# fomalhautb/KM-BART

Hardware: AMD Instinct MI355X
Metric: train_tokens_per_sec (higher is better)
Workload: dtype bf16

## Files before the change

km-bart_amd/csrc/gemm.hip:

```cpp
#include <algorithm>
#include <cstdio>
#include <cstdlib>
#include <cstring>
#include <map>
#include <tuple>
#include <vector>
#include <type_traits>
#include "common.h"
#include "diag.h"
#include "kernels.h"

#ifdef KMB_GEMM_STAMP
#ifndef KMB_STAMP_SLOTS
#define KMB_STAMP_SLOTS 8
#endif
__device__ unsigned long long* g_kmb_stamps = nullptr;
extern "C" int kmb_debug_set_stamps(void* p) {
  return (int)hipMemcpyToSymbol(HIP_SYMBOL(g_kmb_stamps), &p, sizeof(p));
}
#define KMB_STAMP(i)                                                                                   \
  do {                                                                                                 \
    if (g_kmb_stamps != nullptr && threadIdx.x == 0)                                                   \
      g_kmb_stamps[(size_t)blockIdx.x * KMB_STAMP_SLOTS + (i)] = __builtin_amdgcn_s_memrealtime();                   \
  } while (0)
// ... 1033 lines not shown
      __builtin_amdgcn_sched_group_barrier(0x100, NDA, 3);
      __builtin_amdgcn_sched_group_barrier(0x008, 2, 3);
#pragma unroll
      for (int q = 0; q < 2; ++q) {
        __builtin_amdgcn_sched_group_barrier(0x010, 2, 3);
        __builtin_amdgcn_sched_group_barrier(0x008, 6, 3);
      }
    }
    __builtin_amdgcn_sched_barrier(0);
  };
  using Yes = std::true_type;
  using No = std::false_type;
  int t = 0;
  for (; t + 2 < nt; ++t) kstep(t, Yes{}, Yes{});
  if (t + 1 < nt) { kstep(t, No{}, Yes{}); ++t; }
  kstep(t, No{}, No{});
  __syncthreads();
  KMB_STAMP(2);
  KMB_STAMP_VALUE(5, kmb_wait_ticks);
  if (KMB_DIAG_BIT(p.tile_order, 512)) {
    float keep = 0.f;
#pragma unroll
    for (int i = 0; i < 8; ++i)
#pragma unroll
      for (int j = 0; j < 4; ++j) keep += acc[i][j][0];
    if (keep == 1.2345e30f) p.out_bf16[0] = 0;
    return;
  }
  float* ef = reinterpret_cast<float*>(smem);
  for (int h = 0; h < 2; ++h) {
    if ((wn >> 1) == h) {
#pragma unroll
      for (int i = 0; i < 8; ++i)
#pragma unroll
        for (int j = 0; j < 4; ++j)
#pragma unroll
          for (int q = 0; q < 4; ++q)
            ef[(wm * 128 + i * 16 + g * 4 + q) * EPI_LD + (wn & 1) * 64 + j * 16 + r] = acc[i][j][q];
    }
    __syncthreads();
    if (h == 0) KMB_STAMP(3);
    gemm_epilogue_phase2<512, false>(p, ef, reinterpret_cast<float*>(smem + 2 * EPI_BYTES), tid, row0, col0 + h * 128, slice);
    __syncthreads();
  }
  KMB_STAMP(4);
}


#ifndef KMB_GEMM_DEVICE_ONLY
constexpr int VR = 320, VN = 256;
constexpr int VK = 32;
constexpr int V_A = VR * VK * 2;
constexpr int V_STG = (VR + VN) * VK * 2;
constexpr int V_NSTG = 4;
constexpr int LDS_VOC = V_NSTG * V_STG;

template <bool STATS>
__global__ __launch_bounds__(512) void gemm_kernel_allrows(const KmbGemm p, float* __restrict__ stats) {
  extern __shared__ __attribute__((aligned(16))) char smem[];
  const int tid = threadIdx.x;
  const int lane = tid & 63, wave = __builtin_amdgcn_readfirstlane(tid >> 6);
  const int wm = wave >> 2, wn = wave & 3;
  const int r = lane & 15, g = lane >> 4;
  const int col0 = (int)blockIdx.x * VN;
  f32x4 acc[10][4];
#pragma unroll
  for (int i = 0; i < 10; ++i)
#pragma unroll
    for (int j = 0; j < 4; ++j) acc[i][j] = f32x4{0.f, 0.f, 0.f, 0.f};
  const int ns = p.K / VK;
  const int prow = lane >> 2, pchunk = (lane & 3) ^ ((0 - (lane >> 4)) & 3);
  uint32_t offA[3], offB[2];
#pragma unroll
  for (int i = 0; i < 3; ++i) {
    const int row = (wave + 8 * i) * 16 + prow;
    const int grow = row < p.M ? row : p.M - 1;
    offA[i] = (uint32_t)((grow * p.lda + pchunk * 8) * 2);
  }
#pragma unroll
  for (int i = 0; i < 2; ++i) {
    const int col = col0 + (2 * wave + i) * 16 + prow;
    const int gcol = col < p.N ? col : p.N - 1;
    offB[i] = (uint32_t)(((gcol - col0) * p.ldb + pchunk * 8) * 2);
  }
  auto uniform_ptr = [](const char* ptr) {
    const uint64_t a = reinterpret_cast<uint64_t>(ptr);
    const uint32_t lo = __builtin_amdgcn_readfirstlane((uint32_t)a);
    const uint32_t hi = __builtin_amdgcn_readfirstlane((uint32_t)(a >> 32));
    return reinterpret_cast<const char*>(((uint64_t)hi << 32) | lo);
  };
  const char* const gA = reinterpret_cast<const char*>(p.A);
  const char* const gB = reinterpret_cast<const char*>(p.B) + (size_t)col0 * p.ldb * 2;
  auto dma_stage = [&](int s) {
    char* st = smem + (s & (V_NSTG - 1)) * V_STG;
    const char* ga = uniform_ptr(gA + (size_t)s * VK * 2);
    const char* gb = uniform_ptr(gB + (size_t)s * VK * 2);
    dma_piece(ga, offA[0], st + wave * 1024);
    dma_piece(ga, offA[1], st + (wave + 8) * 1024);
    if (wave < 4) dma_piece(ga, offA[2], st + (wave + 16) * 1024);
    dma_piece(gb, offB[0], st + V_A + (2 * wave) * 1024);
    dma_piece(gb, offB[1], st + V_A + (2 * wave + 1) * 1024);
  };
  KMB_STAMP(0);
  KMB_STAMP_ID();
#ifdef KMB_GEMM_STAMP
  const uint64_t kmb_c0 = __builtin_amdgcn_s_memtime(), kmb_r0 = __builtin_amdgcn_s_memrealtime();
#endif
  dma_stage(0);
  if (ns > 1) dma_stage(1);
  if (ns > 2) dma_stage(2);
  const int frag_off = r * 64 + ((g ^ ((0 - (r >> 2)) & 3)) << 4);
  for (int s = 0; s < ns; ++s) {
    const int newer = ns - 1 - s;
    if (wave < 4) {
      if (newer >= 2) __builtin_amdgcn_s_waitcnt(0x0F7A);
      else if (newer == 1) __builtin_amdgcn_s_waitcnt(0x0F75);
      else __builtin_amdgcn_s_waitcnt(0x0F70);
    } else {
      if (newer >= 2) __builtin_amdgcn_s_waitcnt(0x0F78);
      else if (newer == 1) __builtin_amdgcn_s_waitcnt(0x0F74);
      else __builtin_amdgcn_s_waitcnt(0x0F70);
    }
    __builtin_amdgcn_s_barrier();
    if (s == 0) KMB_STAMP(1);
    if (s == ns / 2) KMB_STAMP(3);
    const bool more = s + 3 < ns;
    char* nst = smem + ((s + 3) & (V_NSTG - 1)) * V_STG;
    const char* ga = uniform_ptr(gA + (size_t)(s + 3) * VK * 2);
    const char* gb = uniform_ptr(gB + (size_t)(s + 3) * VK * 2);
    const char* cur = smem + (s & (V_NSTG - 1)) * V_STG + frag_off;
    bf16x8 fb[4], fa[10];
#pragma unroll
    for (int j = 0; j < 4; ++j) fb[j] = *reinterpret_cast<const bf16x8*>(cur + V_A + (wn * 4 + j) * 1024);
#pragma unroll
    for (int i = 0; i < 10; ++i) fa[i] = *reinterpret_cast<const bf16x8*>(cur + (wm * 10 + i) * 1024);
#pragma unroll
    for (int i = 0; i < 10; ++i) {
#pragma unroll
      for (int j = 0; j < 4; ++j) acc[i][j] = __builtin_amdgcn_mfma_f32_16x16x32_bf16(fb[j], fa[i], acc[i][j], 0, 0, 0);
      if (more && (i & 1)) {
        if (i == 1) dma_piece(gb, offB[0], nst + V_A + (2 * wave) * 1024);
        if (i == 3) dma_piece(ga, offA[0], nst + wave * 1024);
        if (i == 5) dma_piece(gb, offB[1], nst + V_A + (2 * wave + 1) * 1024);
        if (i == 7) dma_piece(ga, offA[1], nst + (wave + 8) * 1024);
        if (i == 9 && wave < 4) dma_piece(ga, offA[2], nst + (wave + 16) * 1024);
      }
    }
  }
  __syncthreads();
  KMB_STAMP(2);
#ifdef KMB_GEMM_STAMP
  KMB_STAMP_VALUE(5, __builtin_amdgcn_s_memtime() - kmb_c0);
  KMB_STAMP_VALUE(6, __builtin_amdgcn_s_memrealtime() - kmb_r0);
#endif
  if constexpr (!STATS) {
#pragma unroll
    for (int j = 0; j < 4; ++j) {
      const int col = col0 + wn * 64 + j * 16 + g * 4;
      if (col >= p.N) continue;
      f32x4 b4 = {0.f, 0.f, 0.f, 0.f};
      if (p.bias != nullptr) b4 = *reinterpret_cast<const f32x4*>(p.bias + col);
#pragma unroll
      for (int i = 0; i < 10; ++i) {
        const int row = wm * 160 + i * 16 + r;
        if (row < p.M) *reinterpret_cast<f32x4*>(p.out_f32 + (size_t)row * p.ld_out_f32 + col) = acc[i][j] + b4;
      }
    }
  } else {
    float* smax = reinterpret_cast<float*>(smem);
    float* ssum = smax + VR * 4;
    f32x4 b4[4];
    bool inside[4];
#pragma unroll
    for (int j = 0; j < 4; ++j) {
      const int col = col0 + wn * 64 + j * 16 + g * 4;
      inside[j] = col < p.N;
      b4[j] = f32x4{0.f, 0.f, 0.f, 0.f};
      if (p.bias != nullptr && inside[j]) b4[j] = *reinterpret_cast<const f32x4*>(p.bias + col);
    }
    const bool ragged = col0 + VN > p.N;
#pragma unroll
    for (int i = 0; i < 10; ++i) {
      float lm = -INFINITY;
#pragma unroll
      for (int j = 0; j < 4; ++j) {
        acc[i][j] = acc[i][j] + b4[j];
        if (ragged && !inside[j]) acc[i][j] = f32x4{-INFINITY, -INFINITY, -INFINITY, -INFINITY};
        lm = fmaxf(fmaxf(lm, fmaxf(acc[i][j][0], acc[i][j][1])), fmaxf(acc[i][j][2], acc[i][j][3]));
      }
      lm = fmaxf(lm, __shfl_xor(lm, 16, 64));
      lm = fmaxf(lm, __shfl_xor(lm, 32, 64));
      if (g == 0) smax[(wm * 160 + i * 16 + r) * 4 + wn] = lm;
    }
    __syncthreads();
#pragma unroll
    for (int i = 0; i < 10; ++i) {
      const int row = wm * 160 + i * 16 + r;
      const f32x4 m4 = *reinterpret_cast<const f32x4*>(smax + row * 4);
      const float m = fmaxf(fmaxf(m4[0], m4[1]), fmaxf(m4[2], m4[3]));
      float sum = 0.f;
#pragma unroll
      for (int j = 0; j < 4; ++j) {
        if (row < p.M && inside[j])
          *reinterpret_cast<f32x4*>(p.out_f32 + (size_t)row * p.ld_out_f32 + col0 + wn * 64 + j * 16 + g * 4) = acc[i][j];
#pragma unroll
        for (int q = 0; q < 4; ++q) sum += __expf(acc[i][j][q] - m);
      }
      sum += __shfl_xor(sum, 16, 64);
      sum += __shfl_xor(sum, 32, 64);
      if (g == 0) ssum[row * 4 + wn] = sum;
    }
    __syncthreads();
    if (tid < p.M) {
      const f32x4 m4 = *reinterpret_cast<const f32x4*>(smax + tid * 4);
      const f32x4 s4 = *reinterpret_cast<const f32x4*>(ssum + tid * 4);
      float2 ms;
      ms.x = fmaxf(fmaxf(m4[0], m4[1]), fmaxf(m4[2], m4[3]));
      ms.y = (s4[0] + s4[1]) + (s4[2] + s4[3]);
      reinterpret_cast<float2*>(stats)[(size_t)tid * gridDim.x + blockIdx.x] = ms;
    }
  }
  KMB_STAMP(4);
}

#endif

template <bool KC, int NP = 8>
__device__ __forceinline__ void dma_offsets256w4(uint32_t (&off)[NP], int ld, int r0, int R, int wave, int lane) {
#pragma unroll
  for (int i = 0; i < NP; ++i) {
    const int piece = wave * NP + i;
    if (KC) {
      const int row = piece * 8 + (lane >> 3);
      const int c = (lane & 7) ^ ((row >> 1) & 7);
      int grow = r0 + row;
      grow = grow < R ? grow : R - 1;
      off[i] = (uint32_t)(((grow - r0) * ld + c * 8) * 2);
    } else {
      const int krow = piece * 2 + (lane >> 5);
      const int ps = lane & 31;
      const int c32 = (ps >> 1) ^ swz_nkc(krow);
      int m = r0 + c32 * 16 + (ps & 1) * 8;
      const int mlast = ((R - 1) >> 3) << 3;
      m = m < R ? m : mlast;
      off[i] = (uint32_t)((krow * ld + (m - r0)) * 2);
    }
  }
}

constexpr int EPW_BYTES = 16 * 128 * 4;
constexpr int LDS11 = 2 * ST4 + 4 * EPW_BYTES;
constexpr int LDS12 = 2 * (BM4 + 128) * BK * 2 + 4 * EPW_BYTES;

template <int ACT, bool RES, bool CS, bool FAST, int WROWS, int NJ = 8>
__device__ __forceinline__ void v11_epilogue(const KmbGemm& p, f32x4 (&acc)[8][NJ], float* ef, int lane, int r, int g,
                                             int row0w, int col0w) {
  constexpr int WCOLS = NJ * 16;
  constexpr int LDE = WCOLS > 64 ? 128 : 64;
  float csum[8];
#pragma unroll
  for (int e = 0; e < 8; ++e) csum[e] = 0.f;
  float* const wbase = ef + r * LDE;
  const int sw = (r & 7) << 3;
  auto stage = [&](const f32x4 (&a)[NJ]) {
#pragma unroll
    for (int j = 0; j < NJ; ++j) *reinterpret_cast<f32x4*>(wbase + ((j * 16 + g * 4) ^ sw)) = a[j];
    asm volatile("" ::: "memory");
  };
#pragma unroll 1
  for (int i = 0; i < WROWS / 16; ++i) {
    switch (i) {
      case 0: stage(acc[0]); break;
      case 1: stage(acc[1]); break;
      case 2: stage(acc[2]); break;
      case 3: stage(acc[3]); break;
      case 4: stage(acc[4]); break;
      case 5: stage(acc[5]); break;
      case 6: stage(acc[6]); break;
      default: stage(acc[7]); break;
    }
    gemm_epilogue_body<64, (WCOLS > 64), 4, LDE, true, 128, ACT, RES, CS, FAST, true, WCOLS>(p, ef, nullptr, lane, row0w + i * 16,
                                                                                    col0w, csum);
  }
  if (CS && (ACT >= 0 || p.colsum != nullptr)) {
#pragma unroll
    for (int e = 0; e < 8; ++e) {
      csum[e] += __shfl_xor(csum[e], 16);
      csum[e] += __shfl_xor(csum[e], 32);
    }
    if (lane < WCOLS / 8) {
      const int prow = row0w >> 6;
      const int c8 = lane * 8;
#pragma unroll
      for (int e = 0; e < 8; ++e) {
        if (FAST || col0w + c8 + e < p.N) {
          p.colsum[(size_t)prow * p.N + col0w + c8 + e] = csum[e];
          if (WROWS == 128 && (FAST || row0w + 64 < p.M)) p.colsum[(size_t)(prow + 1) * p.N + col0w + c8 + e] = 0.f;
        }
      }
    }
  }
}

template <bool BIAS, bool SCALE, int ACT, bool RES, bool DROP, bool CS, int WROWS, bool F32 = false, int NJ = 8>
__device__ __forceinline__ void v11_epilogue_lean(const KmbGemm& p, f32x4 (&acc)[8][NJ], float* ef, int lane, int r, int g,
                                                  int row0w, int col0w) {
  constexpr int WCOLS = NJ * 16;
  constexpr int CL = WCOLS > 64 ? 16 : 8, RPI = 64 / CL, NIT = 16 / RPI, LDE = WCOLS > 64 ? 128 : 64;
  const int lr = lane / CL;
  const int c8 = ((lane % CL) * 8 < WCOLS) ? (lane % CL) * 8 : WCOLS - 8;
  const int gcol = col0w + c8;
  kmb_f32x2 bias2[4], csum2[4];
#pragma unroll
  for (int e = 0; e < 4; ++e) {
    bias2[e] = BIAS ? kmb_f32x2{p.bias[gcol + 2 * e], p.bias[gcol + 2 * e + 1]} : kmb_f32x2{0.f, 0.f};
    csum2[e] = kmb_f32x2{0.f, 0.f};
  }
  const kmb_f32x2 scale2 = {p.col_scale, p.col_scale};
  const kmb_f32x2 dscale2 = {p.drop_scale, p.drop_scale};
  float* const wbase = ef + r * LDE;
  const int sw = (r & 7) << 2;
  auto stage = [&](const f32x4 (&a)[NJ]) {
#pragma unroll
    for (int j = 0; j < NJ; ++j) *reinterpret_cast<f32x4*>(wbase + ((j * 16 + g * 4) ^ sw)) = a[j];
    asm volatile("" ::: "memory");
  };
  const float* rd[NIT];
#pragma unroll
  for (int it = 0; it < NIT; ++it)
    rd[it] = ef + (lr + RPI * it) * LDE + (c8 ^ (((lr + RPI * it) & 7) << 2));
  const int rd_hi = (lr & 1) ? -4 : 4;
  bf16_t* out = F32 ? nullptr : p.out_bf16 + (size_t)(row0w + lr) * p.ld_out_bf16 + gcol;
  float* out32 = F32 ? p.out_f32 + (size_t)(row0w + lr) * p.ld_out_f32 + gcol : nullptr;
  bf16_t* pre = (ACT == 1 && p.preact != nullptr) ? p.preact + (size_t)(row0w + lr) * p.ld_preact + gcol : nullptr;
  const bf16_t* side = nullptr;
  size_t ld_side = 0;
  if (RES) { side = p.residual + (size_t)(row0w + lr) * p.ld_res + gcol; ld_side = (size_t)p.ld_res; }
  if (ACT == 2) { side = p.aux + (size_t)(row0w + lr) * p.ld_aux + gcol; ld_side = (size_t)p.ld_aux; }
  constexpr bool SIDE = RES || ACT == 2;
  static_assert(!(RES && ACT == 2), "one side stream");
  constexpr bool PAIRS = NIT == 4;
  constexpr int AHEAD = PAIRS ? 2 : 1;
  u32x4 sE[NIT];
  [[maybe_unused]] u32x4 sO[NIT];
  if (SIDE) {
#pragma unroll
    for (int it = 0; it < NIT; ++it) {
      sE[it] = *reinterpret_cast<const u32x4*>(side + (size_t)(RPI * it) * ld_side);
      if constexpr (PAIRS) sO[it] = *reinterpret_cast<const u32x4*>(side + (size_t)(16 + RPI * it) * ld_side);
    }
  }
  float hE[NIT];
  [[maybe_unused]] float hO[NIT];
  const float* shift_base = ACT == 5 ? p.row_shift + row0w + lr : nullptr;
  if constexpr (ACT == 5) {
#pragma unroll
    for (int it = 0; it < NIT; ++it) {
      hE[it] = shift_base[RPI * it];
      if constexpr (PAIRS) hO[it] = shift_base[16 + RPI * it];
    }
  }
  auto stage_chunk = [&](int i) {
    switch (i) {
      case 0: stage(acc[0]); break;
      case 1: stage(acc[1]); break;
      case 2: stage(acc[2]); break;
      case 3: stage(acc[3]); break;
      case 4: stage(acc[4]); break;
      case 5: stage(acc[5]); break;
      case 6: stage(acc[6]); break;
      default: stage(acc[7]); break;
    }
  };
  static_assert((WROWS / 16) % 2 == 0, "chunks are walked in pairs");
  auto chunk = [&](const int i, u32x4 (&sv)[NIT], float (&hv)[NIT]) {
    [[maybe_unused]] float su[SIDE ? NIT : 1][8];
    [[maybe_unused]] float hc[ACT == 5 ? NIT : 1];
    const int ahead = i + AHEAD < WROWS / 16 ? i + AHEAD : WROWS / 16 - 1;
    if (SIDE) {
#pragma unroll
      for (int it = 0; it < NIT; ++it) unpack8(sv[it], su[it]);
      __builtin_amdgcn_sched_barrier(0);
#pragma unroll
      for (int it = 0; it < NIT; ++it) sv[it] = *reinterpret_cast<const u32x4*>(side + (size_t)(16 * ahead + RPI * it) * ld_side);
    }
    if constexpr (ACT == 5) {
#pragma unroll
      for (int it = 0; it < NIT; ++it) hc[it] = hv[it];
#pragma unroll
      for (int it = 0; it < NIT; ++it) asm volatile("" : "+v"(hc[it]));
      __builtin_amdgcn_sched_barrier(0);
#pragma unroll
      for (int it = 0; it < NIT; ++it) hv[it] = shift_base[16 * ahead + RPI * it];
    }
    f32x4 lo4[NIT], hi4[NIT];
#pragma unroll
    for (int it = 0; it < NIT; ++it) {
      lo4[it] = *reinterpret_cast<const f32x4*>(rd[it]);
      hi4[it] = *reinterpret_cast<const f32x4*>(rd[it] + rd_hi);
    }
    asm volatile("" ::: "memory");
    if (i + 1 < WROWS / 16) stage_chunk(i + 1);
#pragma unroll
    for (int it = 0; it < NIT; ++it) {
      const f32x4 lo = lo4[it];
      const f32x4 hi = hi4[it];
      kmb_f32x2 v[4] = {{lo[0], lo[1]}, {lo[2], lo[3]}, {hi[0], hi[1]}, {hi[2], hi[3]}};
#pragma unroll
      for (int e = 0; e < 4; ++e) {
        if (BIAS) v[e] = v[e] + bias2[e];
        if (SCALE) v[e] = v[e] * scale2;
      }
      const size_t roff = (size_t)(16 * i + RPI * it);
      if constexpr (ACT == 5) {
        static_assert(ACT != 5 || WCOLS == 64 || WCOLS == 128, "act 5: 64- or 128-column wave blocks");
        const int grow = row0w + lr + 16 * i + RPI * it;
        const float c = hc[it];
        const kmb_f32x2 c2 = {c, c};
#pragma unroll
        for (int e = 0; e < 4; ++e) v[e] = v[e] - c2;
        if (p.pick_col != nullptr) {
          const int rel = (int)((long long)p.pick_col[grow] - (long long)gcol);
          if (rel >= 0 && rel < 8) {
            float picked = 0.f;
#pragma unroll
            for (int e = 0; e < 4; ++e) {
              if (rel == 2 * e) picked = v[e][0];
              if (rel == 2 * e + 1) picked = v[e][1];
            }
            p.pick_out[grow] = picked;
          }
        }
#pragma unroll
        for (int e = 0; e < 4; ++e) {
          const kmb_f32x2 t = v[e] * 1.4426950408889634f;
          v[e] = kmb_f32x2{__builtin_amdgcn_exp2f(fminf(t[0], 115.f)), __builtin_amdgcn_exp2f(fminf(t[1], 115.f))};
        }
        float sum = (v[0][0] + v[0][1]) + (v[1][0] + v[1][1]) + ((v[2][0] + v[2][1]) + (v[3][0] + v[3][1]));
#pragma unroll
        for (int o = 1; o < CL; o <<= 1) sum += __shfl_xor(sum, o);
        if ((lane % CL) == 0) {
          float* slot = p.row_sums + (size_t)grow * p.row_sums_ld + (col0w >> 6);
          slot[0] = sum;
          if (WCOLS == 128) slot[1] = 0.f;
        }
      } else if (ACT == 1) {
        if (pre != nullptr) {
          kmb_f32x2 dv[4];
#pragma unroll
          for (int e = 0; e < 4; ++e) {
            kmb_f32x2 y;
            gelu_both2(v[e], y, dv[e]);
            v[e] = y;
          }
          const u32x4 pk = {pack2bf(dv[0][0], dv[0][1]), pack2bf(dv[1][0], dv[1][1]), pack2bf(dv[2][0], dv[2][1]), pack2bf(dv[3][0], dv[3][1])};
          KMB_NT_STORE(pk, reinterpret_cast<u32x4*>(pre + roff * p.ld_preact));
        } else {
#pragma unroll
          for (int e = 0; e < 4; ++e) v[e] = gelu2(v[e]);
        }
      } else if (ACT == 2) {
#pragma unroll
        for (int e = 0; e < 4; ++e) v[e] = v[e] * kmb_f32x2{su[it][2 * e], su[it][2 * e + 1]};
      }
      if (DROP) {
        const uint32_t grow = (uint32_t)(row0w + lr + 16 * i + RPI * it);
#pragma unroll
        for (int e = 0; e < 4; ++e) {
          const kmb_f32x2 kept = v[e] * dscale2;
          v[e][0] = drop_keep(p.drop_seed, grow, (uint32_t)(gcol + 2 * e), p.drop_thr16) ? kept[0] : 0.f;
          v[e][1] = drop_keep(p.drop_seed, grow, (uint32_t)(gcol + 2 * e + 1), p.drop_thr16) ? kept[1] : 0.f;
        }
      }
      if (RES) {
#pragma unroll
        for (int e = 0; e < 4; ++e) v[e] = v[e] + kmb_f32x2{su[it][2 * e], su[it][2 * e + 1]};
      }
      if (CS) {
#pragma unroll
        for (int e = 0; e < 4; ++e) csum2[e] = csum2[e] + v[e];
      }
      if (F32) {
        float* o = out32 + roff * p.ld_out_f32;
        KMB_NT_STORE((f32x4{v[0][0], v[0][1], v[1][0], v[1][1]}), reinterpret_cast<f32x4*>(o));
        KMB_NT_STORE((f32x4{v[2][0], v[2][1], v[3][0], v[3][1]}), reinterpret_cast<f32x4*>(o + 4));
      } else {
        const u32x4 pk = {pack2bf(v[0][0], v[0][1]), pack2bf(v[1][0], v[1][1]), pack2bf(v[2][0], v[2][1]), pack2bf(v[3][0], v[3][1])};
#ifdef KMB_PLAIN_FFN_OUT
        if (ACT == 1 || ACT == 2) *reinterpret_cast<u32x4*>(out + roff * p.ld_out_bf16) = pk;
        else KMB_NT_STORE(pk, reinterpret_cast<u32x4*>(out + roff * p.ld_out_bf16));
#else
        KMB_NT_STORE(pk, reinterpret_cast<u32x4*>(out + roff * p.ld_out_bf16));
#endif
      }
    }
  };
  stage_chunk(0);
  if constexpr (PAIRS) {
#pragma unroll 1
    for (int i = 0; i < WROWS / 16; i += 2) {
      chunk(i, sE, hE);
      chunk(i + 1, sO, hO);
    }
  } else {
#pragma unroll 1
    for (int i = 0; i < WROWS / 16; ++i) chunk(i, sE, hE);
  }
  if (CS) {
    float csum[8];
#pragma unroll
    for (int e = 0; e < 4; ++e) { csum[2 * e] = csum2[e][0]; csum[2 * e + 1] = csum2[e][1]; }
#pragma unroll
    for (int e = 0; e < 8; ++e) {
      if (CL == 8) csum[e] += __shfl_xor(csum[e], 8);
      csum[e] += __shfl_xor(csum[e], 16);
      csum[e] += __shfl_xor(csum[e], 32);
    }
    if (lane < CL) {
      const int prow = row0w >> 6;
#pragma unroll
      for (int e = 0; e < 8; ++e) {
        p.colsum[(size_t)prow * p.N + gcol + e] = csum[e];
        if (WROWS == 128) p.colsum[(size_t)(prow + 1) * p.N + gcol + e] = 0.f;
      }
    }
  }
}

template <bool A_KC, bool B_KC, int BNT, int NW = 4>
__global__ __launch_bounds__(NW * 64) __attribute__((amdgpu_waves_per_eu(NW / 4, NW / 4)))
void gemm_kernel_v11(const KmbGemm p, uint32_t* sched, int dyn_first) {
  static_assert(NW == 4 || (NW == 8 && (BNT == 256 || BNT == 192)), "eight waves: 256 x 256 and 256 x 192 tiles only");
  extern __shared__ __attribute__((aligned(16))) char smem[];
  KMB_STAMP(0);
  KMB_STAMP_ID();
  [[maybe_unused]] uint64_t kmb_loop_ticks = 0, kmb_epi_ticks = 0, kmb_wait_ticks = 0, kmb_drain_ticks = 0;
  const int tid = threadIdx.x;
  const int lane = tid & 63, wave = __builtin_amdgcn_readfirstlane(tid >> 6);
  constexpr int WN = NW == 8 ? 4 : BNT == 128 ? 1 : 2, WM = NW / WN, WROWS = BM4 / WM, MH = WROWS / 64;
  constexpr int WCOLS = BNT / WN, NJ = WCOLS / 16;
  constexpr int BIMG = (BNT == 192 && !B_KC) ? 256 : BNT;
  constexpr int NPA = 32 / NW;
  constexpr int NPB = BIMG / 32 * 4 / NW;
  constexpr int STG = (BM4 + BIMG) * BK * 2;
  const int wm = wave / WN, wn = wave % WN;
  const int r = lane & 15, g = lane >> 4;
  const int tiles_n = (p.N + BNT - 1) / BNT;
  const int tiles_m = (p.M + BM4 - 1) / BM4;
  const int ntiles = tiles_m * tiles_n;
  constexpr int CB = 8;
  const bool col_blocks = (p.tile_order & 8) != 0 && tiles_n > CB;
  const int cb_full = tiles_n / CB;
  auto decode_tile = [&](int t, int& tm, int& tn) {
    if (!col_blocks) { tm = t / tiles_n; tn = t - tm * tiles_n; return; }
    const int blk = t / (CB * tiles_m);
    if (blk < cb_full) {
      const int rem = t - blk * (CB * tiles_m);
      tm = rem / CB; tn = blk * CB + (rem - tm * CB);
    } else {
      const int wl = tiles_n - cb_full * CB;
      const int rem = t - cb_full * (CB * tiles_m);
      tm = rem / wl; tn = cb_full * CB + (rem - tm * wl);
    }
  };
  const int pf_sharers = col_blocks ? CB : tiles_n;
  const bool xcd_ranges = (p.tile_order & 1) != 0;
  const int per = xcd_ranges ? (int)gridDim.x >> 3 : (int)gridDim.x;
  const int xcd = (int)blockIdx.x & 7, loc = (int)blockIdx.x >> 3;
  const int tq = ntiles >> 3, trem = ntiles & 7;
  const int range0 = !xcd_ranges ? 0 : xcd < trem ? xcd * (tq + 1) : trem * (tq + 1) + (xcd - trem) * tq;
  const int range1 = !xcd_ranges ? ntiles : range0 + tq + (xcd < trem ? 1 : 0);
  const int first = xcd_ranges ? range0 + loc : (int)blockIdx.x;
  const bool dyn = sched != nullptr;
  uint32_t* const my_ctr = sched + (xcd_ranges ? xcd : 0);
  auto retire = [&]() {
    if (dyn && tid == 0) {
      if (atomicAdd(sched + 8, 1u) == gridDim.x - 1u) {
#pragma unroll
        for (int i = 0; i < 9; ++i) sched[i] = 0u;
      }
    }
  };
  int* const next_slot = reinterpret_cast<int*>(smem + 2 * STG);
  constexpr int PFW = NW - 1;
  const unsigned touch_lds = kmb_lds_addr(smem + 2 * STG + PFW * (WCOLS > 64 ? EPW_BYTES : EPW_BYTES / 2) + 2048);
  uint32_t fetched = 0u;
  const int dyn_base = (dyn && dyn_first) ? range0 : range0 + per;
  int first_tile = first;
  if (dyn && dyn_first) {
    if (tid == 0) *next_slot = range0 + (int)atomicAdd(my_ctr, 1u);
    __syncthreads();
    first_tile = __builtin_amdgcn_readfirstlane(*next_slot);
    __syncthreads();
  }
  if (first_tile >= range1) { retire(); return; }
#if defined(KMB_GEMM_STAMP) && KMB_STAMP_SLOTS >= 12
  const uint64_t kmb_c0 = __builtin_amdgcn_s_memtime(), kmb_r0 = __builtin_amdgcn_s_memrealtime();
#endif
#ifdef KMB_DIAG
  if (const int stg = (p.tile_order >> 16) & 255) {
    const int q = ((int)blockIdx.x >> 3) & 3;
    for (int i = 0; i < q * stg; ++i) __builtin_amdgcn_s_sleep(18);
  }
#endif
  const int nt = p.K / BK;
  constexpr int A_BYTES = BM4 * BK * 2;
  const size_t stepA = A_KC ? (size_t)BK * 2 : (size_t)BK * p.lda * 2;
  const size_t stepB = B_KC ? (size_t)BK * 2 : (size_t)BK * p.ldb * 2;
  auto uniform_ptr = [](const char* ptr) {
    const uint64_t a = reinterpret_cast<uint64_t>(ptr);
    const uint32_t lo = __builtin_amdgcn_readfirstlane((uint32_t)a);
    const uint32_t hi = __builtin_amdgcn_readfirstlane((uint32_t)(a >> 32));
    return reinterpret_cast<const char*>(((uint64_t)hi << 32) | lo);
  };

  uint32_t offA[NPA], offB[NPB];
  const char *gA_d, *gB_d;
  int tile_d = first_tile, td = 0;
#ifndef KMB_V11_PREFETCH
#define KMB_V11_PREFETCH 1
#endif
#ifndef KMB_V11_PFD
#define KMB_V11_PFD 2
#endif
  constexpr int KMB_PFD = KMB_V11_PFD;
  constexpr bool PF_ON = KMB_V11_PREFETCH != 0 && A_KC;
  const bool pf_rt = (p.tile_order & 2) != 0;
  uint32_t pf_off = 0u, pfn_off = 0u;
  const char* pfn_base = reinterpret_cast<const char*>(p.A);
  bool pf_pending = false, pfn_ok = false;
  auto pf_row_offset = [&](int tn, int row0) {
    int share = (BM4 + pf_sharers - 1) / pf_sharers;
    share = share > 64 ? 64 : share;
    int prow = tn * share + (lane < share ? lane : 0);
    prow = prow < BM4 ? prow : BM4 - 1;
    prow = row0 + prow < p.M ? prow : 0;
    return (uint32_t)prow * (uint32_t)p.lda * 2u;
  };
  auto set_dma_tile = [&](int tile) {
    int tm, tn;
    decode_tile(tile, tm, tn);
    const int row0 = tm * BM4, col0 = tn * BNT;
    if (PF_ON) {
      pf_off = pf_row_offset(col_blocks ? tn % CB : tn, row0);
      const int tx = tile + per;
      pfn_ok = tx < range1;
      if (pfn_ok) {
        int tmx, tnx;
        decode_tile(tx, tmx, tnx);
        pfn_off = pf_row_offset(col_blocks ? tnx % CB : tnx, tmx * BM4);
        pfn_base = uniform_ptr(reinterpret_cast<const char*>(p.A) + (size_t)tmx * BM4 * p.lda * 2);
      }
    }
    dma_offsets256w4<A_KC, NPA>(offA, p.lda, row0, p.M, wave, lane);
    if constexpr (BNT == 128) dma_offsets<B_KC>(offB, p.ldb, col0, p.N, wave, lane);
    else dma_offsets256w4<B_KC, NPB>(offB, p.ldb, col0, p.N, wave, lane);
    gA_d = uniform_ptr(reinterpret_cast<const char*>(p.A) + (A_KC ? (size_t)row0 * p.lda * 2 : (size_t)row0 * 2));
    gB_d = uniform_ptr(reinterpret_cast<const char*>(p.B) + (B_KC ? (size_t)col0 * p.ldb * 2 : (size_t)col0 * 2));
  };
  int tile_next = first_tile;
  auto advance_cursor = [&]() {
    if (td == nt) {
      td = 0;
      tile_next = dyn ? __builtin_amdgcn_readfirstlane(*next_slot) : tile_d + per;
      if (tile_next < range1) tile_d = tile_next;
      set_dma_tile(tile_d);
    }
  };
  char* const dstA = smem + wave * (NPA * 1024);
  char* const dstB = smem + A_BYTES + wave * (NPB * 1024);
#ifndef KMB_V11_SPLIT
#define KMB_V11_SPLIT 1
#endif
  constexpr int NA3 = KMB_V11_SPLIT == 3 ? NPA / 2 : NPA;
  constexpr int NB3 = KMB_V11_SPLIT == 0 ? NPB : 0;
  constexpr int NB0 = KMB_V11_SPLIT == 0 ? 0 : KMB_V11_SPLIT == 2 ? NPB / 2 : NPB;
  constexpr int NB1 = NPB - NB3 - NB0;
  constexpr int P3 = (NA3 + NB3) / 2, P0 = (NPA - NA3 + NB0) / 2, P1 = NB1 / 2;
  auto dma_a = [&](int buf, int lo, int hi) {
    char* da = dstA + buf * STG;
#ifndef KMB_V11_NODMA
#pragma unroll
    for (int i = 0; i < NPA; ++i) {
#ifdef KMB_A_NT
      if (i >= lo && i < hi) { if constexpr (A_KC) dma_piece_nt(gA_d, offA[i], da + i * 1024); else dma_piece(gA_d, offA[i], da + i * 1024); }
#else
      if (i >= lo && i < hi) dma_piece(gA_d, offA[i], da + i * 1024);
#endif
    }
#endif
    if (hi == NPA && lo < hi) gA_d = uniform_ptr(gA_d + stepA);
  };
  auto dma_b = [&](int buf, int lo, int hi) {
    char* db = dstB + buf * STG;
#ifndef KMB_V11_NODMA
#pragma unroll
    for (int i = 0; i < NPB; ++i)
      if (i >= lo && i < hi) dma_piece(gB_d, offB[i], db + i * 1024);
#endif
    if (hi == NPB && lo < hi) {
      gB_d = uniform_ptr(gB_d + stepB);
      ++td;
    }
  };
  auto dma_stage_a = [&](int buf) { dma_a(buf, 0, NPA); };
  auto dma_stage_b = [&](int buf, int) { dma_b(buf, 0, NPB); };

  constexpr int NDA = A_KC ? 4 : 8;
  constexpr int NDB = B_KC ? NJ : 2 * NJ;
  constexpr int NM = 4 * NJ;
  bf16x8 fa[2][4], fb[2][NJ];
  f32x4 acc[8][NJ];
  constexpr bool REMAT = NW == 8;
  const int rm_ka = r * 128 + ((g ^ ((r >> 1) & 7)) << 4);
  const int rm_sw = ((r >> 2) & 3) | ((g & 1) << 2);
  const int rm_l = (g * 8 + (r >> 2)) * (BIMG * 2) + ((r & 3) << 3);
  const int rm_nb = rm_l | (rm_sw << 5);
  const int rm_na = ((g * 8 + (r >> 2)) * (BM4 * 2) + ((r & 3) << 3)) | (rm_sw << 5);
#ifndef KMB_TR_BUILTIN
  constexpr bool TRASM = (BNT == 256 || KMB_TR_ALL) && !(A_KC && B_KC);
#else
  constexpr bool TRASM = false;
#endif
  auto tr_read = [&](const char* ptr) {
#ifndef KMB_TR_BUILTIN
    if constexpr (TRASM) return kmb_tr_read_asm(ptr);
    else
#endif
    return __builtin_amdgcn_ds_read_tr16_b64_v4i16((__attribute__((address_space(3))) s16x4*)ptr);
  };
  auto read_a = [&](const char* stage, int kk, int half, bf16x8 (&dst)[4]) {
    if constexpr (REMAT && A_KC) {
      int c = rm_ka;
      asm volatile("" : "+v"(c));
      const char* base = stage + (c ^ (kk << 6)) + (wm * (MH * 4) + half * 4) * 2048;
#pragma unroll
      for (int i = 0; i < 4; ++i) dst[i] = *reinterpret_cast<const bf16x8*>(base + i * 2048);
    } else if constexpr (REMAT) {
      int c = rm_na;
      asm volatile("" : "+v"(c));
#pragma unroll
      for (int i = 0; i < 4; ++i) {
        const char* pj = stage + kk * (32 * BM4 * 2) + (c ^ ((wm * (MH * 4) + half * 4 + i) << 5));
#pragma unroll
        for (int hh = 0; hh < 2; ++hh) {
          const s16x4 t = tr_read(pj + hh * (4 * BM4 * 2));
          dst[i][hh * 4 + 0] = t[0]; dst[i][hh * 4 + 1] = t[1]; dst[i][hh * 4 + 2] = t[2]; dst[i][hh * 4 + 3] = t[3];
        }
      }
    } else {
#pragma unroll
      for (int i = 0; i < 4; ++i) dst[i] = read_frag3<A_KC, BM4, TRASM>(stage, wm * (MH * 4) + half * 4 + i, kk, r, g);
    }
  };
  auto read_b = [&](const char* stage, int kk, bf16x8 (&dst)[NJ]) {
    if constexpr (REMAT && B_KC) {
      int c = rm_ka;
      asm volatile("" : "+v"(c));
      const char* base = stage + A_BYTES + (c ^ (kk << 6)) + (wn * NJ) * 2048;
#pragma unroll
      for (int j = 0; j < NJ; ++j) dst[j] = *reinterpret_cast<const bf16x8*>(base + j * 2048);
    } else if constexpr (REMAT) {
      int c = rm_nb;
      asm volatile("" : "+v"(c));
#pragma unroll
      for (int j = 0; j < NJ; ++j) {
        const char* pj = stage + A_BYTES + kk * (32 * BIMG * 2) + (c ^ ((wn * NJ + j) << 5));
#pragma unroll
        for (int hh = 0; hh < 2; ++hh) {
          const s16x4 t = tr_read(pj + hh * (4 * BIMG * 2));
          dst[j][hh * 4 + 0] = t[0]; dst[j][hh * 4 + 1] = t[1]; dst[j][hh * 4 + 2] = t[2]; dst[j][hh * 4 + 3] = t[3];
        }
      }
    } else {
#pragma unroll
      for (int j = 0; j < NJ; ++j) dst[j] = read_frag3<B_KC, BIMG, TRASM>(stage + A_BYTES, wn * NJ + j, kk, r, g);
    }
  };
#ifdef KMB_V11_MFMA32_TIMING
  f32x16 acc32[4][4];
  static_assert(NJ == 8, "timing experiment: 128-column wave blocks only");
  auto mma = [&](int half, const bf16x8 (&a)[4], const bf16x8 (&b)[8]) {
#pragma unroll
    for (int ii = 0; ii < 2; ++ii)
#pragma unroll
      for (int jj = 0; jj < 4; ++jj)
#pragma unroll
        for (int ks = 0; ks < 2; ++ks)
          acc32[half * 2 + ii][jj] = __builtin_amdgcn_mfma_f32_32x32x16_bf16(b[jj * 2 + ks], a[ii * 2 + ks], acc32[half * 2 + ii][jj], 0, 0, 0);
  };
#define KMB_MF(n) ((n) / 2)
#else
  auto mma = [&](int half, const bf16x8 (&a)[4], const bf16x8 (&b)[NJ]) {
#pragma unroll
    for (int i = 0; i < 4; ++i)
#pragma unroll
      for (int j = 0; j < NJ; ++j)
        acc[half * 4 + i][j] = __builtin_amdgcn_mfma_f32_16x16x32_bf16(b[j], a[i], acc[half * 4 + i][j], 0, 0, 0);
  };
#define KMB_MF(n) (n)
#endif

  set_dma_tile(tile_d);
  if (PF_ON && pf_rt && wave == PFW) {
#pragma unroll
    for (int i = 2; i < 2 + KMB_PFD; ++i) {
      if (i < nt) {
        const char* pbase = uniform_ptr(gA_d + (size_t)i * stepA);
        KMB_L2_TOUCH(pf_off, pbase, touch_lds);
// ... 915 lines not shown
```

km-bart_amd/csrc/gemm_lean.hip:

```cpp
#define KMB_GEMM_DEVICE_ONLY
#include "gemm.hip"

namespace {

constexpr int LN_STG = (256 + 256) * BK * 2;
constexpr int LN_A = 256 * BK * 2;
constexpr int LN_EPW = 16 * 64 * 4;
constexpr int LN_LDS = 2 * LN_STG + 8 * LN_EPW;

enum { LN_BIAS = 0, LN_BIAS_RES = 1, LN_PLAIN = 2, LN_GELU = 3, LN_DGELU_CS = 4, LN_CE = 5 };

__device__ __forceinline__ const char* ln_uniform(const char* ptr) {
  const uint64_t a = reinterpret_cast<uint64_t>(ptr);
  const uint32_t lo = (uint32_t)__builtin_amdgcn_readfirstlane((uint32_t)a);
  const uint32_t hi = (uint32_t)__builtin_amdgcn_readfirstlane((uint32_t)(a >> 32));
  return reinterpret_cast<const char*>(((uint64_t)hi << 32) | lo);
}

template <bool B_KC, int EC>
__global__ __launch_bounds__(512) __attribute__((amdgpu_waves_per_eu(2, 2))) void gemm_kernel_lean(const KmbGemm p, uint32_t* sched, int dyn_first) {
  extern __shared__ __attribute__((aligned(16))) char smem[];
  const int tid = threadIdx.x;
  const int lane = tid & 63, wave = __builtin_amdgcn_readfirstlane(tid >> 6);
  const int wm = wave >> 2, wn = wave & 3;
  const int r = lane & 15, g = lane >> 4;
  constexpr int NJ = 4;
  const int tiles_n = p.N / 256, tiles_m = p.M / 256;
  const int ntiles = tiles_m * tiles_n;
  constexpr int CB = 8;
  const bool col_blocks = (p.tile_order & 8) != 0 && tiles_n > CB;
  const int cb_full = tiles_n / CB;
  auto decode_tile = [&](int t, int& tm, int& tn) {
    if (!col_blocks) { tm = t / tiles_n; tn = t - tm * tiles_n; return; }
    const int blk = t / (CB * tiles_m);
    if (blk < cb_full) {
      const int rem = t - blk * (CB * tiles_m);
      tm = rem / CB; tn = blk * CB + (rem - tm * CB);
    } else {
      const int wl = tiles_n - cb_full * CB;
      const int rem = t - cb_full * (CB * tiles_m);
      tm = rem / wl; tn = cb_full * CB + (rem - tm * wl);
    }
  };
  const int per = (int)gridDim.x >> 3;
  const int xcd = (int)blockIdx.x & 7, loc = (int)blockIdx.x >> 3;
  const int tq = ntiles >> 3, trem = ntiles & 7;
  const int range0 = xcd < trem ? xcd * (tq + 1) : trem * (tq + 1) + (xcd - trem) * tq;
  const int range1 = range0 + tq + (xcd < trem ? 1 : 0);
  const int nt = p.K / BK;
  const bool dyn = sched != nullptr;
  uint32_t* const my_ctr = sched + xcd;
  auto retire = [&]() {
    if (dyn && tid == 0) {
      if (atomicAdd(sched + 8, 1u) == gridDim.x - 1u) {
#pragma unroll
        for (int i = 0; i < 9; ++i) sched[i] = 0u;
      }
    }
  };
  int* const next_slot = reinterpret_cast<int*>(smem + 2 * LN_STG);
  const int dyn_base = (dyn && dyn_first) ? range0 : range0 + per;
  int first_tile = range0 + loc;
  if (dyn && dyn_first) {
    if (tid == 0) *next_slot = range0 + (int)atomicAdd(my_ctr, 1u);
    __syncthreads();
    first_tile = __builtin_amdgcn_readfirstlane(*next_slot);
    __syncthreads();
  }
  if (first_tile >= range1) { retire(); return; }

  constexpr int NPW = 4;
  constexpr bool TRASM = KMB_TR_ALL && !B_KC;
  uint32_t offA[NPW], offB[NPW];
  dma_offsets256w4<true, 4>(offA, p.lda, 0, 1 << 30, wave, lane);
  dma_offsets256w4<B_KC, 4>(offB, p.ldb, 0, 1 << 30, wave, lane);
  const size_t stepB = B_KC ? (size_t)BK * 2 : (size_t)BK * p.ldb * 2;
  const char *gA_d, *gB_d;
  int tile_d = first_tile, td = 0;
  int tile_next = first_tile;
  constexpr int LN_PFD = 2;
#ifdef KMB_LN_NOTOUCH
  constexpr int TCH = 0;
#else
  constexpr int TCH = 1;
#endif
  const int sharers = col_blocks ? CB : tiles_n;
  const int pf_share = (256 + sharers - 1) / sharers;
  const int pf_gs = (pf_share + 7) >> 3;
  const char *gA_tile, *gA_nx;
  int pf_rows = 0, pf_rows_nx = 0;
  auto set_dma_tile = [&](int tile) {
    int tm, tn;
    decode_tile(tile, tm, tn);
    gA_d = ln_uniform(reinterpret_cast<const char*>(p.A) + (size_t)tm * 256 * p.lda * 2);
    gB_d = ln_uniform(reinterpret_cast<const char*>(p.B) + (B_KC ? (size_t)tn * 256 * p.ldb * 2 : (size_t)tn * 256 * 2));
    gA_tile = gA_d;
    pf_rows = (col_blocks ? tn % CB : tn) * pf_share;
    const int tx = (!dyn && tile + per < range1) ? tile + per : tile;
    decode_tile(tx, tm, tn);
    gA_nx = ln_uniform(reinterpret_cast<const char*>(p.A) + (size_t)tm * 256 * p.lda * 2);
    pf_rows_nx = (col_blocks ? tn % CB : tn) * pf_share;
  };
  const unsigned touch_lds = kmb_lds_addr(smem + 2 * LN_STG + wave * LN_EPW + 2048);
  auto touch = [&](int ahead) {
    const int ps = td + ahead;
    const bool nx = ps >= nt;
    const char* sbase = ln_uniform((nx ? gA_nx : gA_tile) + (size_t)(nx ? ps - nt : ps) * (BK * 2));
    int row = wave * pf_gs + (lane < pf_gs ? lane : pf_gs - 1);
    row = row < pf_share ? row : pf_share - 1;
    row += nx ? pf_rows_nx : pf_rows;
    row = row < 256 ? row : 255;
    const uint32_t voff = (uint32_t)row * (uint32_t)p.lda * 2u;
    KMB_L2_TOUCH(voff, sbase, touch_lds);
  };
  auto dma_stage = [&](char* stage) {
    char* da = stage + wave * 4096;
    char* db = stage + LN_A + wave * 4096;
#pragma unroll
    for (int i = 0; i < 4; ++i) dma_piece(gA_d, offA[i], da + i * 1024);
#pragma unroll
    for (int i = 0; i < 4; ++i) dma_piece(gB_d, offB[i], db + i * 1024);
    gA_d = ln_uniform(gA_d + BK * 2);
    gB_d = ln_uniform(gB_d + stepB);
  };
  auto advance_cursor = [&]() {
    if (++td == nt) {
      td = 0;
      tile_next = dyn ? __builtin_amdgcn_readfirstlane(*next_slot) : tile_d + per;
      if (tile_next < range1) tile_d = tile_next;
      set_dma_tile(tile_d);
    }
  };

  bf16x8 fa[2][4], fb[2][NJ];
  f32x4 acc[8][NJ];
  auto read_a = [&](const char* st, int kk, int half, bf16x8 (&d)[4]) {
#pragma unroll
    for (int i = 0; i < 4; ++i) d[i] = read_frag3<true, 256>(st, wm * 8 + half * 4 + i, kk, r, g);
  };
  [[maybe_unused]] uint32_t bbase[NJ];
  if constexpr (TRASM) {
    const int krow0 = g * 8 + (r >> 2);
#pragma unroll
    for (int j = 0; j < NJ; ++j) bbase[j] = (uint32_t)(LN_A + krow0 * 512 + (((wn * NJ + j) ^ swz_nkc(krow0)) << 5) + ((r & 3) << 3));
  }
  auto read_b = [&](const char* st, auto kk_c, bf16x8 (&d)[NJ]) {
    constexpr int kk = decltype(kk_c)::value;
    if constexpr (TRASM) {
#ifndef KMB_TR_BUILTIN
      const uint32_t sb = (uint32_t)(uintptr_t)(__attribute__((address_space(3))) const char*)st;
#pragma unroll
      for (int j = 0; j < NJ; ++j) {
        const uint32_t a = sb + bbase[j];
        const s16x4 t0 = kmb_tr_read_asm_off<kk * 32 * 512>(a);
        const s16x4 t1 = kmb_tr_read_asm_off<(kk * 32 + 4) * 512>(a);
        d[j][0] = t0[0]; d[j][1] = t0[1]; d[j][2] = t0[2]; d[j][3] = t0[3];
        d[j][4] = t1[0]; d[j][5] = t1[1]; d[j][6] = t1[2]; d[j][7] = t1[3];
      }
#endif
    } else {
#pragma unroll
      for (int j = 0; j < NJ; ++j) d[j] = read_frag3<B_KC, 256, false>(st + LN_A, wn * NJ + j, kk, r, g);
    }
  };
  using K0 = std::integral_constant<int, 0>;
  using K1 = std::integral_constant<int, 1>;
  auto mma = [&](int half, const bf16x8 (&a)[4], const bf16x8 (&b)[NJ]) {
#pragma unroll
    for (int i = 0; i < 4; ++i)
#pragma unroll
      for (int j = 0; j < NJ; ++j)
        acc[half * 4 + i][j] = __builtin_amdgcn_mfma_f32_16x16x32_bf16(b[j], a[i], acc[half * 4 + i][j], 0, 0, 0);
  };
  constexpr int NDA = 4, NDB = B_KC ? NJ : 2 * NJ;
  auto kstep = [&](char* cur, const char* nxt, auto last_c, int w, int ntouch) {
    constexpr bool LAST = decltype(last_c)::value;
    if constexpr (TRASM) KMB_TR_SYNC();
    read_a(cur, 0, 1, fa[1]);
    mma(0, fa[0], fb[0]);
#pragma unroll
    for (int q = 0; q < NDA; ++q) { __builtin_amdgcn_sched_group_barrier(0x008, 2, 0); __builtin_amdgcn_sched_group_barrier(0x100, 1, 0); __builtin_amdgcn_sched_group_barrier(0x008, 2, 0); }
    __builtin_amdgcn_sched_barrier(0);
    if constexpr (TRASM) KMB_TR_SYNC();
    read_b(cur, K1{}, fb[1]);
    read_a(cur, 1, 0, fa[0]);
    mma(1, fa[1], fb[0]);
#pragma unroll
    for (int q = 0; q < 8; ++q) { __builtin_amdgcn_sched_group_barrier(0x008, 2, 1); __builtin_amdgcn_sched_group_barrier(0x100, (NDB + NDA + 7) / 8, 1); }
    __builtin_amdgcn_sched_barrier(0);
    if constexpr (TRASM) KMB_TR_SYNC();
    read_a(cur, 1, 1, fa[1]);
    mma(0, fa[0], fb[1]);
#pragma unroll
    for (int q = 0; q < NDA; ++q) { __builtin_amdgcn_sched_group_barrier(0x008, 2, 2); __builtin_amdgcn_sched_group_barrier(0x100, 1, 2); __builtin_amdgcn_sched_group_barrier(0x008, 2, 2); }
    __builtin_amdgcn_sched_barrier(0);
    if (LAST || w == 0) __builtin_amdgcn_s_waitcnt(0x0070);
    else if (w == 1) __builtin_amdgcn_s_waitcnt(0x0071);
    else __builtin_amdgcn_s_waitcnt(0x0072);
    __builtin_amdgcn_s_barrier();
    __builtin_amdgcn_s_waitcnt(0xC07F);
    __builtin_amdgcn_sched_barrier(0);
    if constexpr (!LAST) {
      read_b(nxt, K0{}, fb[0]);
      read_a(nxt, 0, 0, fa[0]);
    }
    dma_stage(cur);
    mma(1, fa[1], fb[1]);
    if constexpr (!LAST) {
#pragma unroll
      for (int q = 0; q < 8; ++q) { __builtin_amdgcn_sched_group_barrier(0x008, 2, 3); __builtin_amdgcn_sched_group_barrier(0x100, (NDB + NDA + 7) / 8, 3); }
    }
    __builtin_amdgcn_sched_barrier(0);
    if constexpr (!LAST && TCH != 0) {
      if (ntouch >= 1) touch(LN_PFD);
      if (ntouch >= 2) touch(LN_PFD + 2);
      __builtin_amdgcn_sched_barrier(0);
    }
    advance_cursor();
  };
  using Yes = std::true_type;
  using No = std::false_type;
  set_dma_tile(tile_d);
  dma_stage(smem);
  if constexpr (TCH != 0) touch(LN_PFD);
  advance_cursor();
  dma_stage(smem + LN_STG);
  if constexpr (TCH != 0) touch(LN_PFD);
  advance_cursor();
  __builtin_amdgcn_s_waitcnt(TCH ? 0x0F7A : 0x0F78);
  __builtin_amdgcn_s_barrier();
  read_b(smem, K0{}, fb[0]);
  read_a(smem, 0, 0, fa[0]);

  float* const ef = reinterpret_cast<float*>(smem + 2 * LN_STG + wave * LN_EPW);
  int it = 0;
  uint32_t fetched = 0u;
  for (int tile = first_tile; tile < range1; tile = tile_next) {
#pragma unroll
    for (int i = 0; i < 8; ++i)
#pragma unroll
      for (int j = 0; j < NJ; ++j) acc[i][j] = f32x4{0.f, 0.f, 0.f, 0.f};
    int w = 0;
    for (int t = 0; t + 1 < nt; ++t, ++it) {
      if (dyn && t == 1 && tid == 0) fetched = atomicAdd(my_ctr, 1u);
      if (dyn && t == 3 && tid == 0) *next_slot = dyn_base + (int)fetched;
      const int ntouch = TCH == 0 ? 0 : t + 4 < nt ? 1 : t + 2 < nt ? 2 : 0;
      kstep(smem + (it & 1) * LN_STG, smem + ((it + 1) & 1) * LN_STG, No{}, w, ntouch);
      w = ntouch;
    }
    kstep(smem + (it & 1) * LN_STG, smem + ((it + 1) & 1) * LN_STG, Yes{}, 0, 0);
    ++it;
    if constexpr (TRASM) KMB_TR_SYNC();
    if (KMB_DIAG_BIT(p.tile_order, 512)) {
#pragma unroll
      for (int i = 0; i < 8; ++i)
#pragma unroll
        for (int j = 0; j < NJ; ++j) asm volatile("" ::"v"(acc[i][j]));
    } else {
      int tm, tn;
      decode_tile(tile, tm, tn);
      const int row0w = tm * 256 + wm * 128, col0w = tn * 256 + wn * 64;
      const bool hs = col0w < p.col_scale_n, hd = p.drop_thr16 != 0u, hr = p.residual != nullptr;
#define KMB_LN_LEAN(B, S, A, R, D, C) v11_epilogue_lean<B, S, A, R, D, C, 128, false, NJ>(p, acc, ef, lane, r, g, row0w, col0w)
      if constexpr (EC == LN_BIAS) { if (hs) KMB_LN_LEAN(true, true, 0, false, false, false); else KMB_LN_LEAN(true, false, 0, false, false, false); }
      if constexpr (EC == LN_BIAS_RES) { if (hd) KMB_LN_LEAN(true, false, 0, true, true, false); else KMB_LN_LEAN(true, false, 0, true, false, false); }
      if constexpr (EC == LN_PLAIN) { if (hr) KMB_LN_LEAN(false, false, 0, true, false, false); else KMB_LN_LEAN(false, false, 0, false, false, false); }
      if constexpr (EC == LN_GELU) KMB_LN_LEAN(true, false, 1, false, false, false);
      if constexpr (EC == LN_DGELU_CS) KMB_LN_LEAN(false, false, 2, false, false, true);
      if constexpr (EC == LN_CE) KMB_LN_LEAN(true, false, 5, false, false, false);
#undef KMB_LN_LEAN
    }
    __builtin_amdgcn_sched_barrier(0);
    read_b(smem + (it & 1) * LN_STG, K0{}, fb[0]);
    read_a(smem + (it & 1) * LN_STG, 0, 0, fa[0]);
  }
  if constexpr (TRASM) KMB_TR_SYNC();
  __builtin_amdgcn_s_waitcnt(0x0F70);
  retire();
}

int ln_class(const KmbGemm& p) {
  const bool hb = p.bias != nullptr, hr = p.residual != nullptr, hd = p.drop_thr16 != 0u, hc = p.colsum != nullptr;
  const bool hs = p.col_scale_n > 0;
  if (p.act == 0 && hb && !hr && !hd && !hc) return LN_BIAS;
  if (p.act == 0 && hb && hr && !hc && !hs) return LN_BIAS_RES;
  if (p.act == 0 && !hb && !hd && !hc && !hs) return LN_PLAIN;
  if (p.act == 1 && hb && !hr && !hd && !hc && !hs) return LN_GELU;
  if (p.act == 2 && !hb && !hr && !hd && hc && !hs) return LN_DGELU_CS;
  if (p.act == 5 && hb && !hr && !hd && !hc && !hs) return LN_CE;
  return -1;
}

template <bool B_KC>
hipError_t ln_launch_layout(int ec, const KmbGemm& p, dim3 grid, hipStream_t stream, uint32_t* sched, int dyn_first) {
#define KMB_LN_CASE(E)                                                                                                          \
  case E: {                                                                                                                     \
    static bool attr = false;                                                                                                   \
    if (!attr) {                                                                                                                \
      hipError_t e = hipFuncSetAttribute((const void*)gemm_kernel_lean<B_KC, E>, hipFuncAttributeMaxDynamicSharedMemorySize, LN_LDS); \
      if (e != hipSuccess) return e;                                                                                            \
      attr = true;                                                                                                              \
    }                                                                                                                           \
    hipLaunchKernelGGL((gemm_kernel_lean<B_KC, E>), grid, dim3(512), LN_LDS, stream, p, sched, dyn_first);                                         \
    break;                                                                                                                      \
  }
  switch (ec) {
    KMB_LN_CASE(LN_BIAS)
    KMB_LN_CASE(LN_BIAS_RES)
    KMB_LN_CASE(LN_PLAIN)
    KMB_LN_CASE(LN_GELU)
    KMB_LN_CASE(LN_DGELU_CS)
    KMB_LN_CASE(LN_CE)
    default: return hipErrorInvalidValue;
  }
#undef KMB_LN_CASE
  return hipGetLastError();
}

}

bool kmb_gemm_lean_ok(const KmbGemm& p) {
  if (!p.a_kc || p.split_k > 1 || (p.K % BK) != 0 || p.K / BK < 5) return false;
  if ((p.M % 256) != 0 || (p.N % 256) != 0) return false;
  if ((long)(p.M / 256) * (p.N / 256) < 128) return false;
  if (p.out_bf16 == nullptr || p.out_f32 != nullptr || p.beta != 0.f) return false;
  if (p.col_scale_n > 0 && (p.col_scale_n % 64) != 0) return false;
  if (p.act == 5 && (p.row_shift == nullptr || p.row_sums == nullptr)) return false;
  if ((long)p.lda * 2 * 256 >= (1L << 31) || (long)p.ldb * 2 * 256 >= (1L << 31)) return false;
  return ln_class(p) >= 0;
}

hipError_t kmb_gemm_lean_launch(const KmbGemm& p, hipStream_t stream, uint32_t* sched, int dyn_first) {
  if (!kmb_gemm_lean_ok(p)) return hipErrorInvalidValue;
  if (p.K / BK < 8) sched = nullptr;
  const long tiles = (long)(p.M / 256) * (p.N / 256);
  const dim3 grid(tiles >= 256 ? 256u : (unsigned)(tiles & ~7L));
  const int ec = ln_class(p);
  return p.b_kc ? ln_launch_layout<true>(ec, p, grid, stream, sched, dyn_first) : ln_launch_layout<false>(ec, p, grid, stream, sched, dyn_first);
}
```

Baseline: 2.178 million.

## Peel final epilogue chunks and relax vmcnt waits across tile boundaries

Adds a PEEL option to the lean epilogue so the last chunk pair skips the redundant side and shift prefetches, and enables it in the lean GEMM kernel. The first k-step of each later tile now waits with a larger vmcnt (16 or 32, depending on whether the epilogue issues one or two output streams), so the previous tile's epilogue stores need not drain before the next tile's mainloop barrier. This cuts wasted loads and store-drain stalls at tile boundaries. The risk is a wrong count, which could let LDS stage data be read before its DMA has landed.

```diff
diff --git a/km-bart_amd/csrc/gemm.hip b/km-bart_amd/csrc/gemm.hip
--- a/km-bart_amd/csrc/gemm.hip
+++ b/km-bart_amd/csrc/gemm.hip
@@ -1359,7 +1359,7 @@
   }
 }
 
-template <bool BIAS, bool SCALE, int ACT, bool RES, bool DROP, bool CS, int WROWS, bool F32 = false, int NJ = 8>
+template <bool BIAS, bool SCALE, int ACT, bool RES, bool DROP, bool CS, int WROWS, bool F32 = false, int NJ = 8, bool PEEL = false>
 __device__ __forceinline__ void v11_epilogue_lean(const KmbGemm& p, f32x4 (&acc)[8][NJ], float* ef, int lane, int r, int g,
                                                   int row0w, int col0w) {
   constexpr int WCOLS = NJ * 16;
@@ -1430,25 +1430,30 @@
     }
   };
   static_assert((WROWS / 16) % 2 == 0, "chunks are walked in pairs");
-  auto chunk = [&](const int i, u32x4 (&sv)[NIT], float (&hv)[NIT]) {
+  auto chunk = [&](const int i, u32x4 (&sv)[NIT], float (&hv)[NIT], auto pf_c) {
+    constexpr bool PF = decltype(pf_c)::value;
     [[maybe_unused]] float su[SIDE ? NIT : 1][8];
     [[maybe_unused]] float hc[ACT == 5 ? NIT : 1];
     const int ahead = i + AHEAD < WROWS / 16 ? i + AHEAD : WROWS / 16 - 1;
     if (SIDE) {
 #pragma unroll
       for (int it = 0; it < NIT; ++it) unpack8(sv[it], su[it]);
-      __builtin_amdgcn_sched_barrier(0);
-#pragma unroll
-      for (int it = 0; it < NIT; ++it) sv[it] = *reinterpret_cast<const u32x4*>(side + (size_t)(16 * ahead + RPI * it) * ld_side);
+      if constexpr (PF) {
+        __builtin_amdgcn_sched_barrier(0);
+#pragma unroll
+        for (int it = 0; it < NIT; ++it) sv[it] = *reinterpret_cast<const u32x4*>(side + (size_t)(16 * ahead + RPI * it) * ld_side);
+      }
     }
     if constexpr (ACT == 5) {
 #pragma unroll
       for (int it = 0; it < NIT; ++it) hc[it] = hv[it];
 #pragma unroll
       for (int it = 0; it < NIT; ++it) asm volatile("" : "+v"(hc[it]));
-      __builtin_amdgcn_sched_barrier(0);
-#pragma unroll
-      for (int it = 0; it < NIT; ++it) hv[it] = shift_base[16 * ahead + RPI * it];
+      if constexpr (PF) {
+        __builtin_amdgcn_sched_barrier(0);
+#pragma unroll
+        for (int it = 0; it < NIT; ++it) hv[it] = shift_base[16 * ahead + RPI * it];
+      }
     }
     f32x4 lo4[NIT], hi4[NIT];
 #pragma unroll
@@ -1553,15 +1558,23 @@
     }
   };
   stage_chunk(0);
+  using Pf = std::true_type;
+  using NoPf = std::false_type;
+  constexpr int NCH = WROWS / 16;
   if constexpr (PAIRS) {
 #pragma unroll 1
-    for (int i = 0; i < WROWS / 16; i += 2) {
-      chunk(i, sE, hE);
-      chunk(i + 1, sO, hO);
+    for (int i = 0; i + (PEEL ? 2 : 0) < NCH; i += 2) {
+      chunk(i, sE, hE, Pf{});
+      chunk(i + 1, sO, hO, Pf{});
+    }
+    if constexpr (PEEL) {
+      chunk(NCH - 2, sE, hE, NoPf{});
+      chunk(NCH - 1, sO, hO, NoPf{});
     }
   } else {
 #pragma unroll 1
-    for (int i = 0; i < WROWS / 16; ++i) chunk(i, sE, hE);
+    for (int i = 0; i + (PEEL ? 1 : 0) < NCH; ++i) chunk(i, sE, hE, Pf{});
+    if constexpr (PEEL) chunk(NCH - 1, sE, hE, NoPf{});
   }
   if (CS) {
     float csum[8];
diff --git a/km-bart_amd/csrc/gemm_lean.hip b/km-bart_amd/csrc/gemm_lean.hip
--- a/km-bart_amd/csrc/gemm_lean.hip
+++ b/km-bart_amd/csrc/gemm_lean.hip
@@ -7,6 +7,8 @@
 constexpr int LN_A = 256 * BK * 2;
 constexpr int LN_EPW = 16 * 64 * 4;
 constexpr int LN_LDS = 2 * LN_STG + 8 * LN_EPW;
+
+constexpr int ln_vmcnt(int n) { return (n & 15) | ((n >> 4) << 14) | 0x0070; }
 
 enum { LN_BIAS = 0, LN_BIAS_RES = 1, LN_PLAIN = 2, LN_GELU = 3, LN_DGELU_CS = 4, LN_CE = 5 };
 
@@ -194,10 +196,13 @@
 #pragma unroll
     for (int q = 0; q < NDA; ++q) { __builtin_amdgcn_sched_group_barrier(0x008, 2, 2); __builtin_amdgcn_sched_group_barrier(0x100, 1, 2); __builtin_amdgcn_sched_group_barrier(0x008, 2, 2); }
     __builtin_amdgcn_sched_barrier(0);
-    if (LAST || w == 0) __builtin_amdgcn_s_waitcnt(0x0070);
-    else if (w == 1) __builtin_amdgcn_s_waitcnt(0x0071);
-    else __builtin_amdgcn_s_waitcnt(0x0072);
+    if (LAST || w == 0) __builtin_amdgcn_s_waitcnt(ln_vmcnt(0));
+    else if (w == 1) __builtin_amdgcn_s_waitcnt(ln_vmcnt(1));
+    else if (w == 2) __builtin_amdgcn_s_waitcnt(ln_vmcnt(2));
+    else if (w == 16) __builtin_amdgcn_s_waitcnt(ln_vmcnt(16));
+    else __builtin_amdgcn_s_waitcnt(ln_vmcnt(32));
     __builtin_amdgcn_s_barrier();
+    asm volatile("" ::: "memory");
     __builtin_amdgcn_s_waitcnt(0xC07F);
     __builtin_amdgcn_sched_barrier(0);
     if constexpr (!LAST) {
@@ -233,6 +238,9 @@
   read_a(smem, 0, 0, fa[0]);
 
   float* const ef = reinterpret_cast<float*>(smem + 2 * LN_STG + wave * LN_EPW);
+  const bool two = (EC == LN_GELU && p.preact != nullptr) || EC == LN_DGELU_CS || EC == LN_BIAS_RES || EC == LN_CE ||
+                   (EC == LN_PLAIN && p.residual != nullptr);
+  const int tail = KMB_DIAG_BIT(p.tile_order, 512) ? 0 : two ? 32 : 16;
   int it = 0;
   uint32_t fetched = 0u;
   for (int tile = first_tile; tile < range1; tile = tile_next) {
@@ -240,7 +248,7 @@
     for (int i = 0; i < 8; ++i)
 #pragma unroll
       for (int j = 0; j < NJ; ++j) acc[i][j] = f32x4{0.f, 0.f, 0.f, 0.f};
-    int w = 0;
+    int w = tile == first_tile ? 0 : tail;
     for (int t = 0; t + 1 < nt; ++t, ++it) {
       if (dyn && t == 1 && tid == 0) fetched = atomicAdd(my_ctr, 1u);
       if (dyn && t == 3 && tid == 0) *next_slot = dyn_base + (int)fetched;
@@ -261,7 +269,7 @@
       decode_tile(tile, tm, tn);
       const int row0w = tm * 256 + wm * 128, col0w = tn * 256 + wn * 64;
       const bool hs = col0w < p.col_scale_n, hd = p.drop_thr16 != 0u, hr = p.residual != nullptr;
-#define KMB_LN_LEAN(B, S, A, R, D, C) v11_epilogue_lean<B, S, A, R, D, C, 128, false, NJ>(p, acc, ef, lane, r, g, row0w, col0w)
+#define KMB_LN_LEAN(B, S, A, R, D, C) v11_epilogue_lean<B, S, A, R, D, C, 128, false, NJ, true>(p, acc, ef, lane, r, g, row0w, col0w)
       if constexpr (EC == LN_BIAS) { if (hs) KMB_LN_LEAN(true, true, 0, false, false, false); else KMB_LN_LEAN(true, false, 0, false, false, false); }
       if constexpr (EC == LN_BIAS_RES) { if (hd) KMB_LN_LEAN(true, false, 0, true, true, false); else KMB_LN_LEAN(true, false, 0, true, false, false); }
       if constexpr (EC == LN_PLAIN) { if (hr) KMB_LN_LEAN(false, false, 0, true, false, false); else KMB_LN_LEAN(false, false, 0, false, false, false); }
```

After: 2.181 million (median of 6 runs). About the same (+0.1%).
